# mdw771/beyond_dof

Hardware: AMD Instinct MI355X
Metric: multislice fwd+adjoint slice-steps/s (full Adam iteration: rotation, forward, loss, adjoint, gradient exchange, regulariser+Adam) (higher is better)
Workload: dtype f32

## Files before the change

### beyond_dof_amd/_lib.py

```python
import ctypes
import os
import sys

import numpy as np

_HERE = os.path.dirname(os.path.abspath(__file__))
LIB_PATH = os.environ.get('BDOF_LIB') or os.path.join(_HERE, 'libbdof.so')

DET_NONE, DET_NEAR, DET_FAR = 0, 1, 2
VARIANT_NUMPY_SKIP_LAST, VARIANT_TF_ALL = 0, 1
LOSS_LSQ, LOSS_POISSON = 0, 1
CFG_GRAD, CFG_GENERIC, CFG_NO_RESIDENT, CFG_ALWAYS_RESIDENT, CFG_RECOMPUTE, CFG_NO_GROT, CFG_ADJOINT64 = 1, 2, 4, 8, 16, 32, 64
K_ROW_FWD, K_COL_PROP, K_ROW_BWD, K_LOSS, K_ROT_ADJ, K_ADAM = range(6)
KERNEL_CLASS_NAMES = ['row_fwd', 'col_prop', 'row_bwd', 'loss', 'rot_adjoint', 'adam']

_c_int_p = ctypes.POINTER(ctypes.c_int)
_c_float_p = ctypes.POINTER(ctypes.c_float)
_vp = ctypes.c_void_p

_SIGNATURES = {
    'bdof_ctx_create': (ctypes.c_int, [ctypes.POINTER(_vp), ctypes.c_int, _vp]),
    'bdof_ctx_destroy': (None, [_vp]),
    'bdof_last_error': (ctypes.c_char_p, [_vp]),
    'bdof_sync': (ctypes.c_int, [_vp]),
# ... 61 lines not shown
    'bdof_grot': (_vp, [_vp]),
    'bdof_tape_slot': (_vp, [_vp, ctypes.c_int]),
    'bdof_modulation_table': (ctypes.c_int, [_vp, ctypes.POINTER(_vp), ctypes.POINTER(ctypes.c_size_t), ctypes.POINTER(ctypes.c_double)]),
    'bdof_rotation_adjoint': (ctypes.c_int, [_vp, ctypes.c_int, _vp, _vp, ctypes.c_int, ctypes.c_float]),
    'bdof_rotation_adjoint_rows': (ctypes.c_int, [_vp, ctypes.c_int, _vp, _vp, ctypes.c_int, ctypes.c_int, ctypes.c_int, ctypes.c_float]),
    'bdof_rotate_bilinear': (ctypes.c_int, [_vp, _vp, ctypes.c_int, ctypes.c_int, ctypes.c_int, _vp, ctypes.c_int, _vp]),
    'bdof_set_object_bilinear': (ctypes.c_int, [_vp, _vp, ctypes.c_int, ctypes.c_int, ctypes.c_int, _vp, ctypes.c_int, ctypes.c_int]),
    'bdof_rotate_bilinear_adjoint': (ctypes.c_int, [_vp, _vp, ctypes.c_int, ctypes.c_int, ctypes.c_int, _vp, ctypes.c_int, _vp, ctypes.c_int, ctypes.c_int, ctypes.c_int, ctypes.c_float]),
    'bdof_window_rotation_adjoint': (ctypes.c_int, [_vp, ctypes.c_int, ctypes.c_int, _vp, _vp, _vp, ctypes.c_int, ctypes.c_float]),
    'bdof_adam_step': (ctypes.c_int, [_vp, _vp, _vp, _vp, _vp, _vp, _vp, ctypes.c_int, ctypes.c_int, ctypes.c_int]
                       + [ctypes.c_float] * 8 + [ctypes.c_int, ctypes.c_int]),
    'bdof_adam_step_slab': (ctypes.c_int, [_vp, _vp, _vp, _vp, _vp, _vp, _vp, ctypes.c_int, ctypes.c_int, ctypes.c_int]
                            + [ctypes.c_float] * 8 + [ctypes.c_int] * 4),
    'bdof_rotation_adjoint_adam': (ctypes.c_int, [_vp, ctypes.c_int, _vp, _vp, ctypes.c_int, ctypes.c_int, ctypes.c_int, ctypes.c_float,
                                                  _vp, _vp, _vp, _vp, _vp, ctypes.c_int, ctypes.c_int, ctypes.c_int]
                                   + [ctypes.c_float] * 8 + [ctypes.c_int, ctypes.c_int]),
    'bdof_regularizer_value': (ctypes.c_int, [_vp, _vp, ctypes.c_int, ctypes.c_int, ctypes.c_int, ctypes.POINTER(ctypes.c_double)]),
    'bdof_mask_shrink': (ctypes.c_int, [_vp, _vp, _vp, ctypes.c_size_t, ctypes.c_float]),
    'bdof_gather_fields': (ctypes.c_int, [_vp, _vp, _vp, _vp, ctypes.c_int, ctypes.c_size_t]),
    'bdof_set_streams': (ctypes.c_int, [_vp, ctypes.c_int]),
    'bdof_batch_groups': (ctypes.c_int, [_vp, ctypes.c_int]),
    'bdof_set_sweep_fusion': (ctypes.c_int, [_vp, ctypes.c_int]),
    'bdof_sweep_fused': (ctypes.c_int, [_vp]),
    'bdof_profile_enable': (ctypes.c_int, [_vp, ctypes.c_int]),
    'bdof_profile_read': (ctypes.c_int, [_vp, ctypes.c_int, _c_int_p, ctypes.POINTER(ctypes.c_double)]),
    'bdof_malloc': (ctypes.c_int, [ctypes.POINTER(_vp), ctypes.c_size_t]),
    'bdof_device_mem': (ctypes.c_int, [_vp, ctypes.POINTER(ctypes.c_size_t), ctypes.POINTER(ctypes.c_size_t)]),
    'bdof_ctx_malloc': (ctypes.c_int, [_vp, ctypes.POINTER(_vp), ctypes.c_size_t]),
    'bdof_comm_unique_id': (ctypes.c_int, [_vp, ctypes.c_size_t]),
    'bdof_comm_create': (ctypes.c_int, [ctypes.POINTER(_vp), ctypes.c_int, ctypes.c_int, ctypes.c_int, _vp, ctypes.c_size_t]),
    'bdof_comm_destroy': (None, [_vp]),
    'bdof_comm_last_error': (ctypes.c_char_p, [_vp]),
    'bdof_comm_size': (ctypes.c_int, [_vp]),
    'bdof_comm_rank': (ctypes.c_int, [_vp]),
    'bdof_allreduce_grad': (ctypes.c_int, [_vp, _vp, _vp, ctypes.c_size_t, _c_int_p]),
    'bdof_reduce_scatter_grad': (ctypes.c_int, [_vp, _vp, _vp, ctypes.c_size_t, _c_int_p]),
    'bdof_allgather_volume': (ctypes.c_int, [_vp, _vp, _vp, ctypes.c_size_t, _c_int_p]),
    'bdof_bcast_volume': (ctypes.c_int, [_vp, _vp, _vp, ctypes.c_size_t, ctypes.c_int, _c_int_p]),
    'bdof_comm_wait': (ctypes.c_int, [_vp, _vp, ctypes.c_int]),
    'bdof_comm_sync': (ctypes.c_int, [_vp]),
    'bdof_free': (ctypes.c_int, [_vp]),
    'bdof_memcpy_h2d': (ctypes.c_int, [_vp, _vp, _vp, ctypes.c_size_t]),
    'bdof_memcpy_d2h': (ctypes.c_int, [_vp, _vp, _vp, ctypes.c_size_t]),
    'bdof_memset': (ctypes.c_int, [_vp, _vp, ctypes.c_int, ctypes.c_size_t]),
    'bdof_memcpy_d2d': (ctypes.c_int, [_vp, _vp, _vp, ctypes.c_size_t]),
}
# ... 153 lines not shown
```

### beyond_dof_amd/csrc/bdof_capi.hip

```cpp
#include <hip/hip_runtime.h>
#include <hip/hip_ext.h>
#include <cmath>
#include <algorithm>
#include <complex>
#include <cstdio>
#include <cstdlib>
#include <cstring>
#include <string>
#include <vector>

#include "../../include/bdof.h"
#include "bdof_steps.h"
#include "bdof_kernels.h"
#include "bdof_conv2.h"
#include "bdof_generic.h"
#include "bdof_field.h"
#include "bdof_conv64.h"
#include "bdof_resident.h"
#include "bdof_comm.h"
#include <rocfft/rocfft.h>
#include <map>
#include <array>

#define BDOF_ERR_ARG (-1)
// ... 70 lines not shown
    DevBuf<double2> cdet64;
    bool resident = false;
    DevBuf<cf> hsT, hdetT, twR, res_carrier;
    DevBuf<cf> pstack, pdet, pdetT;
    DevBuf<double2> pdet64, pdetT64;
    std::map<std::array<int, 4>, PlanPair> plans;
    FftExec fft;
    bool have_h64 = false;
    DevBuf<double2> g64, hs64, hdet64;
};

struct bdof_ctx : Workspace {
    int device = 0;
    hipStream_t stream = nullptr;
    bool own_stream = false;
    hipStream_t side[BDOF_MAX_GROUPS - 1] = {};
    int n_side = -1;
    std::vector<hipStream_t> side_all;
    hipEvent_t ev_fork = nullptr, ev_join[BDOF_MAX_GROUPS - 1] = {};
    hipEvent_t timer[BDOF_N_TIMERS] = {};
    int n_streams = -1;
    int fusion = 0;
    int fused_last = 0;
    int ncu = 256;
    int NY = 0, NX = 0, S = 0, Bmax = 0;
    bool with_grad = false;
    bool recompute = false;
    int tw_dither = 0;
    const float2* obj_src = nullptr;
    const int *adj_off = nullptr, *adj_order = nullptr;
    const cf* range_car = nullptr;
    int range_car_B = 0, range_car_z0 = 0;
    DevBuf<double2> car_scratch;
    hipStream_t aux = nullptr;
    hipEvent_t ev_aux_fork = nullptr, ev_aux_join = nullptr;
    FftExec fft_aux;
    bool aux_pending = false;
    bool c64_tf = false;
    std::complex<double> c64_ksum{1.0, 0.0};
    double c64_k = 0.0;
    int gpsi_B = 0;
    int npartial = 0;
    float k = 0.f;
    float k_fft = 0.f;
    std::complex<double> h00{1.0, 0.0}, hdet00{1.0, 0.0}, a0{0.0, 0.0};
    std::complex<double> cbm1{0.0, 0.0};
// ... 345 lines not shown
    sq_of(c, (unsigned)z, a.sq);
    DISPATCH_N(c->NY, with_bool(a.pz != nullptr, [&](auto PF) {
        BDOF_LAUNCH(ps, (k_row_fwd<N_, false, true, PF, true>), dim3(rows_grid<N_>(c, g.B, c->NX)), dim3(BDOF_THREADS), 0, g.st, a);
    }));
}

static void launch_row_prop(bdof_ctx* c, const Group& g, const cf* in, cf* out, const cf* h, float scale, int conj_h, int key, int cls = BDOF_K_COL_PROP) {
    ProfScope ps(c, cls, g.st, true);
    const unsigned tick = (unsigned)key;
    if (h == c->hs && c->hs_copies > 0) h = c->hs_d + (size_t)(tick % (unsigned)c->hs_copies) * c->NX * c->NY;
    RowPropArgs a{sub_field(c, g, in), sub_field(c, g, out), h, g.B, c->NY, scale, conj_h, tw_of(c, c->twX, c->NX, tick)};
    sq_of(c, tick, a.sq);
    DISPATCH_N(c->NX, {
        BDOF_LAUNCH(ps, (k_row_prop<N_, false>), dim3(rows_grid<N_>(c, g.B, c->NY)), dim3(BDOF_THREADS), 0, g.st, a);
    });
}

static int fused_mode(const bdof_ctx* c) {
    if (c->fusion < 1 || c->sep_copies < 1 || c->recompute || c->bin != 1 || c->pstack || c->range_car) return 0;
    if (c->det_mode == BDOF_DET_FAR || c->obj.xoff || c->obj.yoff || c->gpsi0) return 0;
    if (c->S < 4 || (c->S & 1) || c->NX > 512 || c->NY > 512) return 0;
    return 1;
}
static void launch_slice(bdof_ctx* c, const Group& g, int z, const cf* in, cf* out, cf* phi) {
    ProfScope ps(c, BDOF_K_ROW_FWD, g.st, true);
    const bool xl = (z & 1) != 0;
    const int N = xl ? c->NX : c->NY, R = xl ? c->NY : c->NX;
    const cf* tw = xl ? c->twX : c->twY;
    const cf* h = xl ? c->hx_d : c->hy_d;
    const unsigned lead = (unsigned)(z > 0 ? z - 1 : 0), trail = (unsigned)z, D = (unsigned)c->sep_copies;
    SliceArgs a{sub_field(c, g, in), c->probe, sub_field(c, g, out), sub_field(c, g, phi), sub_obj(c, g), g.B, R, z, carrier_at(c, z), cshift_at(c, z),
                tw_of(c, tw, N, lead), tw_of(c, tw, N, trail), h + (size_t)(lead % D) * N, h + (size_t)(trail % D) * N};
    sq_of(c, lead, a.sq_lead);
    sq_of(c, trail, a.sq_trail);
    if (xl) {
        DISPATCH_N_512(N, BDOF_LAUNCH(ps, (k_slice_x<N_>), dim3(rows_grid<N_>(c, g.B, R)), dim3(BDOF_THREADS), 0, g.st, a));
    } else {
        DISPATCH_N_512(N, with_bool(z == 0, [&](auto FIRST) { with_bool(z == c->S - 2, [&](auto TAIL) {
            BDOF_LAUNCH(ps, (k_slice_y<N_, FIRST, TAIL>), dim3(rows_grid<N_>(c, g.B, R)), dim3(BDOF_THREADS), 0, g.st, a);
        }); }));
    }
}

struct GradTarget {
    float2* grot = nullptr;
    int S_ = 0, z_ = 0;
    cf* gpsi = nullptr;
};
static void launch_row_bwd(bdof_ctx* c, const Group& g, int z, const cf* gin, const cf* tape, cf* gout, int hist = 0, float tape_scale = 1.f,
                           const GradTarget* gt = nullptr) {
    ProfScope ps(c, BDOF_K_ROW_BWD, g.st, true);
    float2* grot = gt && gt->grot ? gt->grot + (size_t)g.b0 * gt->S_ * c->NX * c->NY : c->grot + (size_t)g.b0 * c->S * c->NX * c->NY;
    RowBwdArgs a{sub_field(c, g, gin), hist == 2 ? c->probe : sub_field(c, g, tape), sub_field(c, g, gout),
                 grot, sub_obj(c, g), g.B, c->NX, z, c->k, carrier_at(c, z), tw_of(c, c->twY, c->NY, (unsigned)z),
                 slice_carrier_field(c, z), adj_carrier_at(c, g, steps(c).steps_back(z)), cshift_at(c, z), carrier_phi_at(c, z), tape_scale,
                 gt && gt->gpsi ? sub_field(c, g, gt->gpsi) : (z == 0 ? sub_field<cf>(c, g, c->gpsi0) : nullptr),
                 gt && gt->grot ? gt->S_ : c->S, gt && gt->grot ? gt->z_ : steps(c).first_slice(z)};
    sq_of(c, (unsigned)z, a.sq);
    const int form = a.ac.gcar ? 2 : a.pz ? 1 : 0;
    if (c->bin > 1) {
        DISPATCH_N(c->NY, with_bool(hist == 2, [&](auto H2) { with_int<3>(form, [&](auto FORM) {
            BDOF_LAUNCH(ps, (k_row_bwd<N_, H2 ? 2 : 1, FORM == 1, FORM == 2, true>), dim3(rows_grid<N_>(c, g.B, c->NX)), dim3(BDOF_THREADS), 0, g.st, a);
// ... 40 lines not shown
    a.twiddle = c->twX;
    int grid = 0;
    DISPATCH_N(c->NX, grid = rows_grid<N_>(c, g.B, c->NY); with_bool(meas && loss_is_poisson(c), [&](auto PSN) {
        hipLaunchKernelGGL((k_row_loss<N_, true, true, PSN>), dim3(grid), dim3(BDOF_THREADS), 0, g.st, a);
    }));
    return grid;
}

struct DetRoute {
    bool far;
    const cf* in;
    float in_scale;
    const cf* h;
    const cf* pfield;
};
static DetRoute det_route(const bdof_ctx* c) {
    const bool tf_all = c->variant == BDOF_VARIANT_TF_ALL;
    if (c->det_mode == BDOF_DET_FAR) return DetRoute{true, c->bufA, 1.f, nullptr, c->pdetT};
    if (c->det_mode == BDOF_DET_NONE && !tf_all) return DetRoute{false, c->bufA, 1.f / (float)c->NY, nullptr, c->pdet};
    return DetRoute{false, c->bufB, 1.f, c->det_mode == BDOF_DET_NONE ? c->hs : tf_all ? c->hcomb : c->hdet, c->pdet};
}

enum { TAPE_NONE = 0, TAPE_HISTORY = 1, TAPE_LAST = 2 };
static void forward_sweep(bdof_ctx* c, const Split& split, int tape_mode, bool fused = false) {
    const size_t fld = (size_t)c->Bmax * c->NX * c->NY;
    const DetRoute dr = det_route(c);
    const int nz = n_steps(c);
    for (int z = 0; z < nz; ++z) {
        const cf* in = nullptr;
        if (z > 0) in = tape_mode == TAPE_HISTORY ? c->tape + (size_t)steps(c).tape_read(z) * fld : c->bufB;
        const bool last = z == nz - 1;
        if (fused && last) in = c->tape + (size_t)z * fld;
        if (fused && !last) {
            for (const Group& g : split) {
                launch_slice(c, g, z, (z & 1) ? c->bufA : c->bufB, (z & 1) ? c->bufB : c->bufA, c->tape + (size_t)z * fld);
                if (z == nz - 2) launch_row_prop(c, g, c->bufA, c->tape + (size_t)(nz - 1) * fld, c->hx_rows, 1.f, 0, z, BDOF_K_LOSS);
            }
            continue;
        }
        cf* phi = tape_mode == TAPE_LAST && last ? c->tape : nullptr;
        for (const Group& g : split) {
            if (!last) {
                launch_row_fwd(c, g, z, in, c->bufA, true, phi);
                launch_row_prop(c, g, c->bufA, tape_mode == TAPE_HISTORY ? c->tape + (size_t)steps(c).tape_write(z) * fld : c->bufB, c->hs, 1.f, 0, z);
            } else {
                launch_row_fwd(c, g, z, in, c->bufA, dr.far || dr.h, phi);
                if (dr.h) launch_row_prop(c, g, c->bufA, c->bufB, dr.h, 1.f, 0, z, fused ? BDOF_K_LOSS : BDOF_K_COL_PROP);
            }
        }
    }
}

static void march_back(bdof_ctx* c, const Group& g, int z, int hist, const cf* phi, bool phi_real, bool step, bool march, cf* rc1, cf* rc2,
                       const GradTarget* gt = nullptr) {
    launch_row_bwd(c, g, z, c->bufB, phi, step ? c->bufA : nullptr, hist, 1.f, gt);
    if (step) launch_row_prop(c, g, c->bufA, c->bufB, c->hs, 1.f, 1, z - 1);
    if (march) {
        launch_row_unmod(c, g, z, phi, rc2, phi_real, 1.f);
        launch_row_prop(c, g, rc2, rc1, c->hs, 1.f, 1, z - 1);
    }
}

static void adjoint_sweep(bdof_ctx* c, const Split& split, bool fused) {
    const size_t fld = (size_t)c->Bmax * c->NX * c->NY;
    const int nz = n_steps(c);
    for (int z = nz - 1; z >= 0; --z) {
        const bool top = z == nz - 1;
        for (const Group& g : split) {
            if (c->recompute) {
                march_back(c, g, z, z == 0 ? 2 : top ? 0 : 3, top ? c->tape : c->tape + fld, top, z > 0, z > 1, c->tape + fld, c->tape + 2 * fld);
                continue;
            }
            if (fused) launch_row_bwd(c, g, z, c->bufB, c->tape + (size_t)z * fld, z > 0 ? c->bufA : nullptr, top ? 1 : 0);
            else launch_row_bwd(c, g, z, c->bufB, z > 0 ? c->tape + (size_t)steps(c).tape_read(z) * fld : nullptr, z > 0 ? c->bufA : nullptr, z > 0 ? 1 : 2);
            if (z > 0) launch_row_prop(c, g, c->bufA, c->bufB, c->hs, 1.f, 1, z - 1);
        }
    }
}

static int modulation_room(bdof_ctx* c, size_t n, bool mean) {
    HIPC(c, c->mod.room(n));
    if (mean) HIPC(c, c->cbar_dev.room((size_t)c->ncu * 16 + 1));
    return 0;
}
static int modulation_bound(bdof_ctx* c, size_t at, bool mean) {
    std::complex<double> cb(0.0, 0.0);
    if (mean) {
        double2 m;
        HIPC(c, hipMemcpyAsync(&m, c->cbar_dev + at, sizeof(double2), hipMemcpyDeviceToHost, c->stream));
        HIPC(c, hipStreamSynchronize(c->stream));
        cb = std::complex<double>(m.x, m.y);
        if (c->bin > 1) cb = std::pow(1.0 + cb, c->bin) - 1.0;
    }
// ... 1386 lines not shown
    if (i < nz - 1) {
        launch_loss_real(c, whole(c, B), wave_plane(c, carrier_z(c, i + 1), slice_carrier_field(c, i + 1)), c->tape + (size_t)i * fld, nullptr, false,
                         (cf*)out, nullptr, 1.f, 1.f);
    } else {
        if (!c->last_valid)
            return fail(c, BDOF_ERR_STATE, "the last slice's wave is only kept after bdof_forward(keep_tape=1) with the numpy_skip_last variant");
        launch_loss_real(c, whole(c, B), wave_plane(c, carrier_z(c, nz - 1) * (1.0 + c->cbm1), slice_carrier_field(c, nz - 1)), c->bufA, nullptr, false,
                         (cf*)out, nullptr, 1.f / c->NY, 1.f);
    }
    return launched(c);
}

int bdof_loss_grad(bdof_ctx* c, int B, const int* angle_of_b, const int* xoff, const int* yoff, const float* meas, void* out_wave) {
    int r = check_ready(c, B);
    if (r) return r;
    if (!meas) return BDOF_ERR_ARG;
    if (c->meas_dev && (c->det_mode == BDOF_DET_FAR || c->pstack))
        return fail(c, BDOF_ERR_STATE, "bdof_set_meas_mode(1) needs a real-space detector and a scalar carrier");
    if (!c->with_grad || !c->grot) return fail(c, BDOF_ERR_STATE, "bdof_loss_grad needs bdof_configure(with_grad=1) with the gradient workspace (not flag 32)");
    if ((r = need_angles(c, angle_of_b))) return r;
    if ((r = begin_batch(c, angle_of_b, xoff, yoff, c->k_fft))) return r;
    c->gpsi_src = c->gpsi0;
    c->gpsi_B = B;
    c->fused_last = 0;
    if (use_resident(c, B)) {
        if ((r = resident_run(c, B, meas, out_wave, true))) return r;
        c->tape_valid = c->last_valid = false;
        return 0;
    }
    if (c->generic) {
        if ((r = generic_loss_grad(c, B, meas, out_wave))) return r;
        c->tape_valid = c->last_valid = false;
        c->gpsi_src = c->bufA;
        return launched(c);
    }
    Split split;
    if ((r = split.open(c, B, c->NX, 16))) return r;
    const bool fused = fused_mode(c) != 0;
    c->fused_last = fused ? 1 : 0;
    forward_sweep(c, split, c->recompute ? TAPE_LAST : TAPE_HISTORY, fused);
    c->tape_valid = false;
    c->last_valid = false;
    int npart = 0;
    const DetRoute dr = det_route(c);
    for (const Group& g : split) {
        const DetPlane det = det_plane(c, g, B, dr.pfield);
        if (dr.far) {
            npart += launch_loss_far(c, g, det, dr.in, c->bufB, (cf*)out_wave, meas, 1.f, 1.f, npart);
        } else if (!dr.h) {
            npart += launch_loss_real(c, g, det, dr.in, c->bufB, false, (cf*)out_wave, meas, dr.in_scale, dr.in_scale, npart);
        } else {
            npart += launch_loss_real(c, g, det, dr.in, c->bufA, true, (cf*)out_wave, meas, 1.f, 1.f, npart);
            launch_row_prop(c, g, c->bufA, c->bufB, dr.h, 1.f, 1, n_steps(c) - 1, fused ? BDOF_K_LOSS : BDOF_K_COL_PROP);
        }
    }
    adjoint_sweep(c, split, fused);
    if ((r = split.close(c))) return r;
    hipLaunchKernelGGL(k_sum_partials, dim3(1), dim3(256), 0, c->stream, c->partial, npart,
                       1.0 / ((double)B * c->NX * c->NY), c->loss_dev);
    return launched(c);
}


int bdof_set_conv(bdof_ctx* c, const float* ky, const float* kx, int ks, double e_re, double e_im, double ksum_re,
                  double ksum_im, double k) {
    if (int rb = need_unbinned(c, "bdof_set_conv")) return rb;
    if (!c || !ky || !kx) return BDOF_ERR_ARG;
    if (int r = need_configured(c)) return r;
    if (ks < 1 || ks > BDOF_CONV_MAXK || ks % 2 == 0) return fail(c, BDOF_ERR_ARG, "kernel_size must be odd and <= 33");
    if (c->generic || c->NX % BDOF_CONV_TX || c->NY % BDOF_CONV_TY)
        return fail(c, BDOF_ERR_SIZE, "the conv propagator needs power-of-two wavefields (tiles are 32 x 64)");
    HIPC(c, hipSetDevice(c->device));
    c->c64_tf = false; c->c64_ks = 0;
    for (int i = 0; i < ks; ++i) {
        c->taps.ky[i] = make_float2(ky[2 * i], ky[2 * i + 1]);
        c->taps.kx[i] = make_float2(kx[2 * i], kx[2 * i + 1]);
    }
    c->taps.e = make_float2((float)e_re, (float)e_im);
    c->taps.ks = ks;
// ... 609 lines not shown
    if (!c || !dst || !src || !idx || B < 1) return BDOF_ERR_ARG;
    if (bytes_per_field % 4) return fail(c, BDOF_ERR_SIZE, "bdof_gather_fields: fields must be multiples of 4 bytes");
    HIPC(c, hipSetDevice(c->device));
    if (bytes_per_field % 16) {
        const size_t n4 = bytes_per_field / 4;
        const int gx4 = (int)std::min<size_t>((n4 + 255) / 256, 64);
        hipLaunchKernelGGL(k_gather_fields4, dim3(gx4, B < 1024 ? B : 1024), dim3(256), 0, c->stream, (float*)dst, (const float*)src, idx, B, n4);
        return launched(c);
    }
    const size_t n16 = bytes_per_field / 16;
    const int gx = (int)std::min<size_t>((n16 + 255) / 256, 64);
    hipLaunchKernelGGL(k_gather_fields, dim3(gx, B < 1024 ? B : 1024), dim3(256), 0, c->stream, (float4*)dst, (const float4*)src, idx, B, n16);
    return launched(c);
}

int bdof_set_sweep_fusion(bdof_ctx* c, int mode) {
    if (!c) return BDOF_ERR_ARG;
    if (mode < 0 || mode > 2) return fail(c, BDOF_ERR_ARG, "bdof_set_sweep_fusion: mode must be 0, 1 or 2");
    c->fusion = std::min(mode, 1);
    return 0;
}
int bdof_sweep_fused(bdof_ctx* c) { return c ? c->fused_last : 0; }

int bdof_set_streams(bdof_ctx* c, int n) {
    if (!c) return -1;
    if (n == 0 || n > BDOF_MAX_GROUPS) return fail(c, -2, "bdof_set_streams: n must be -1 or 1..4");
    c->n_streams = n < 0 ? -1 : n;
    return 0;
}

int bdof_batch_groups(bdof_ctx* c, int B) {
    if (!c || B < 1 || !c->NX) return -1;
    if (c->generic) return 1;
    Group g[BDOF_MAX_GROUPS];
    return batch_groups(c, B, c->NX, 16, g);
}

int bdof_profile_enable(bdof_ctx* c, int enable) {
    if (!c) return BDOF_ERR_ARG;
    HIPC(c, hipStreamSynchronize(c->stream));
    prof_collect(c);
    if (enable) { for (int i = 0; i < BDOF_K_COUNT; ++i) { c->prof_ms[i] = 0; c->prof_n[i] = 0; c->prof_seen[i] = 0; } }
    c->prof = enable != 0;
    c->prof_stride = enable > 1 ? enable : 1;
    return 0;
}
// ... 200 lines not shown
```

### beyond_dof_amd/csrc/bdof_kernels.h

```cpp
#pragma once
#include "bdof_fft.h"

#define BDOF_THREADS 512

template <int N> struct RowCfg {
    static constexpr int T = N / 8;
    static constexpr int RPP = BDOF_THREADS / T;
    static constexpr int TILE = RPP > 16 ? RPP : 16;
    static constexpr int PASSES = TILE / RPP;
    static constexpr int NPAD = N + N / 16;
    static constexpr int RS = ((NPAD + 29) / 32) * 32 + 2;
    static constexpr int LDS_CF = TILE * RS;
    static constexpr int MIN_WAVES = N >= 1024 ? 2 : 4;
};

template <int T> struct RowLds {
    cf* base;
    __device__ __forceinline__ int slot(int i) const { return i + (i >> 4); }
    __device__ __forceinline__ cf ld_at(int base_slot, int c) const { return base[base_slot + c + (c >> 4)]; }
    __device__ __forceinline__ void st_at(int base_slot, int c, cf v) { base[base_slot + c + (c >> 4)] = v; }
    __device__ __forceinline__ void sync_w2r() { sync(); }
    __device__ __forceinline__ void sync_r2w() { sync(); }
    __device__ __forceinline__ void sync() {
        if constexpr (T <= 64) {
// ... 747 lines not shown
            cf* pdst = a.phi_out + (size_t)(row0 + r) * NY;
#pragma unroll
            for (int m = 0; m < 8; ++m) pdst[tid + m * C::T] = u[m];
            tw_select(tw, smem_tw[1], smem_tail[1], sqt, tid);
            if constexpr (TAIL) {
                line_fft_partial<NY, -1, 1, false>(u, tw, tid, lds);
            } else {
#pragma unroll
                for (int m = 0; m < 8; ++m) hv[m] = a.h_trail[tid + m * C::T];
                line_fft<NY, -1, 1, false>(u, tw, tid, lds);
#pragma unroll
                for (int m = 0; m < 8; ++m) u[m] = cmul(u[m], hv[m]);
                line_fft_partial<NY, +1, 2, false>(u, tw, tid, lds);
            }
        }
        __syncthreads();
        cf* dst = a.out + (size_t)b * NY * NX + x0;
        if constexpr (TAIL) transposed_tail_mul<NY, -1, 1>(smem, dst, NX, a.h_trail, smem_tail[1], sqt);
        else transposed_tail<NY, +1, 2, false>(smem, dst, NX, 1.f, smem_tail[1], sqt);
        __syncthreads();
    }
}

template <int NX>
__global__ __launch_bounds__(BDOF_THREADS, RowCfg<NX>::MIN_WAVES) void k_slice_x(SliceArgs a) {
    typedef RowCfg<NX> C;
    typedef FftPlan<NX> P;
    __shared__ cf smem[C::LDS_CF];
    __shared__ cf smem_tw[2][FftTw<NX>::LDS_CNT];
    __shared__ cf smem_tail[2][7 * C::T];
    const int tid = threadIdx.x % C::T, rl = threadIdx.x / C::T;
    const float sql[2] = {a.sq_lead[0], a.sq_lead[1]}, sqt[2] = {a.sq_trail[0], a.sq_trail[1]};
    __shared__ int s_src[NX];
    FftTw<NX> tw;
    tw_fill<NX>(a.tw_lead, smem_tw[0], smem_tail[0]);
    tw_fill<NX>(a.tw_trail, smem_tw[1], smem_tail[1]);
    __syncthreads();
    const ObjView o = a.obj;
    const int NY = a.R;
    const int ntiles = a.B * NY / C::TILE;
    for (int tile = blockIdx.x; tile < ntiles; tile += gridDim.x) {
        const int row0 = tile * C::TILE;
        const int b = row0 / NY, y0 = row0 - b * NY;
        const ObjRows rows = obj_rows_of(o, b, a.z, NX);
        cf* const pdst = a.phi_out + (size_t)b * NX * NY;
        const int src_mine = (int)threadIdx.x < NX ? obj_rows_rel(rows, threadIdx.x) : -1;
#pragma nounroll
        for (int pass = 0; pass < C::PASSES; ++pass) {
            const int r = pass * C::RPP + rl;
            RowLds<C::T> lds{smem + r * C::RS};
            cf u[8], hv[8];
            const cf* src = a.in + (size_t)(row0 + r) * NX;
#pragma unroll
            for (int m = 0; m < 8; ++m) u[m] = src[tid + m * C::T];
#pragma unroll
            for (int m = 0; m < 8; ++m) hv[m] = a.h_lead[tid + m * C::T];
            tw_select(tw, smem_tw[0], smem_tail[0], sql, tid);
            line_fft<NX, -1, 1, false>(u, tw, tid, lds);
#pragma unroll
            for (int m = 0; m < 8; ++m) u[m] = cmul(u[m], hv[m]);
            line_fft_partial<NX, +1, 2, false>(u, tw, tid, lds);
        }
        if ((int)threadIdx.x < NX) s_src[threadIdx.x] = src_mine;
        __syncthreads();
        cf v[C::PASSES][8];
#pragma unroll
        for (int pass = 0; pass < C::PASSES; ++pass) {
            const int q = threadIdx.x + pass * BDOF_THREADS;
            const int r = q % C::TILE, j = q / C::TILE;
            RowLds<C::T> lds{smem + r * C::RS};
            const int yg = y0 + r, yc = min(max(yg, 0), o.volNY - 1);
            float2 db[8];
#pragma unroll
            for (int m = 0; m < 8; ++m) {
                const int srel = s_src[j + m * C::T];
                const float2 t = o.vol[(size_t)(rows.plain0 + max(srel, 0)) * o.volNY + yc];
                const bool in = srel >= 0 && yg == yc;
                db[m] = make_float2(in ? t.x : 0.f, in ? t.y : 0.f);
            }
            last_stage<NX, +1, 2, false>(v[pass], j, lds, smem_tail[0], sql);
#pragma unroll
            for (int m = 0; m < 8; ++m) {
                v[pass][m] = modulate_eps_s(v[pass][m], a.carrier, db[m], a.cshift);
                pdst[(unsigned)((j + m * C::T) * NY + yg)] = v[pass][m];
            }
            tw.sq = sqt;
            stage_compute<NX, -1, P::R0, 1, 0, 1, false>(v[pass], tw, j);
        }
        __syncthreads();
#pragma unroll
        for (int pass = 0; pass < C::PASSES; ++pass) {
            const int q = threadIdx.x + pass * BDOF_THREADS;
            const int r = q % C::TILE, j = q / C::TILE;
            RowLds<C::T> lds{smem + r * C::RS};
            stage_write<NX, P::R0, 1>(v[pass], j, lds);
        }
        __syncthreads();
#pragma nounroll
        for (int pass = 0; pass < C::PASSES; ++pass) {
            const int r = pass * C::RPP + rl;
            RowLds<C::T> lds{smem + r * C::RS};
            cf u[8], hv[8];
#pragma unroll
            for (int m = 0; m < 8; ++m) hv[m] = a.h_trail[tid + m * C::T];
            tw_select(tw, smem_tw[1], smem_tail[1], sqt, tid);
            line_fft_rest<NX, -1, 1, false>(u, tw, tid, lds);
#pragma unroll
            for (int m = 0; m < 8; ++m) u[m] = cmul(u[m], hv[m]);
            line_fft_partial<NX, +1, 2, false>(u, tw, tid, lds);
        }
        __syncthreads();
        transposed_tail<NX, +1, 2, false>(smem, a.out + (size_t)b * NX * NY + y0, NY, 1.f, smem_tail[1], sqt);
        __syncthreads();
    }
}

struct AdamArgs {
    const float2* x_old;
    float2* x_new;
    const float2* g;
    float2* m;
    float2* v;
    const float* mask;
    int NXv, NZv, NYv;
    float g_scale;
    float alpha_d, alpha_b, gamma;
    float lr, b1, b2, eps, inv_bc1, inv_bc2;
    float om_b1, om_b2;
    int clip;
    int x0, x1;
};
// ... 941 lines not shown
```

### beyond_dof_amd/engine.py

```python
import ctypes
import os

import numpy as np

from . import _lib
from ._lib import DeviceBuffer
from . import util

_VARIANT = {'numpy_skip_last': _lib.VARIANT_NUMPY_SKIP_LAST, 'tf_all': _lib.VARIANT_TF_ALL}
_LOSS = {'lsq': _lib.LOSS_LSQ, 'poisson': _lib.LOSS_POISSON}


def check_loss(loss_type, poisson_multiplier):
    if loss_type not in _LOSS:
        raise ValueError("loss_type must be 'lsq' or 'poisson'")
    if not float(poisson_multiplier) > 0:
        raise ValueError('poisson_multiplier must be > 0')


def check_poisson_path(loss_type, poisson_multiplier, propagator):
    check_loss(loss_type, poisson_multiplier)
    if loss_type == 'poisson' and propagator != 'fft':
        raise ValueError("loss_type='poisson' runs on the transfer-function propagator (propagator='fft') only")

# ... 387 lines not shown
        self.ctx.check(self.lib.bdof_rotation_adjoint(self.h, B, a.ptr, _lib._ptr(gvol_buf), int(accumulate), float(scale)))
        self.ctx.sync()

    def adam_step(self, x_old, x_new, g, m, v, mask, shape_xzy, i_batch, lr, g_scale=1.0, alpha_d=0.0, alpha_b=0.0,
                  gamma=0.0, b1=0.9, b2=0.999, eps=1e-8, clip=True, slab=None):
        nxv, nzv, nyv = [int(s) for s in shape_xzy]
        x0, nx = (0, nxv) if slab is None else (int(slab[0]), int(slab[1]))
        self.ctx.check(self.lib.bdof_adam_step_slab(self.h, _lib._ptr(x_old), _lib._ptr(x_new), _lib._ptr(g), _lib._ptr(m),
                                                    _lib._ptr(v), _lib._ptr(mask), nxv, nzv, nyv, g_scale, alpha_d, alpha_b,
                                                    gamma, lr, b1, b2, eps, int(i_batch), int(clip), x0, nx))

    def stream_ptr(self):
        return int(self.lib.bdof_stream(self.h) or 0)

    def set_streams(self, n=-1):
        self.ctx.check(self.lib.bdof_set_streams(self.h, int(n)))

    def batch_groups(self, B):
        return int(self.lib.bdof_batch_groups(self.h, int(B)))

    def set_sweep_fusion(self, mode):
        self.ctx.check(self.lib.bdof_set_sweep_fusion(self.h, int(mode)))

    @property
    def sweep_fused(self):
        return int(self.lib.bdof_sweep_fused(self.h))

    def profile_enable(self, on=True, stride=1):
        self.ctx.check(self.lib.bdof_profile_enable(self.h, int(stride) if on else 0))

    def profile_read(self):
        res = {}
        for cls, name in enumerate(_lib.KERNEL_CLASS_NAMES):
            n = ctypes.c_int(0)
            ms = ctypes.c_double(0)
            self.ctx.check(self.lib.bdof_profile_read(self.h, cls, ctypes.byref(n), ctypes.byref(ms)))
            res[name] = (n.value, ms.value)
        return res

    def sync(self):
        self.ctx.sync()
```

### beyond_dof_amd/solver.py

```python
import ctypes
import os

import numpy as np

from . import _lib
from ._lib import DeviceBuffer
from . import util
from .comm import PseudoComm
from .engine import MultisliceEngine, RESIDENT_SIZES, check_poisson_path, check_binning_path


class _VolumeSolver(object):

    lookahead = 2

    def _init_volume(self):
        shape = (self.dim_x, self.dim_z, self.dim_y, 2)
        self.x = [DeviceBuffer.zeros(self.ctx, shape, np.float32), DeviceBuffer.zeros(self.ctx, shape, np.float32)]
        self.cur = 0
        self.g = DeviceBuffer.zeros(self.ctx, shape, np.float32)
        self.m = DeviceBuffer.zeros(self.ctx, shape, np.float32)
        self.v = DeviceBuffer.zeros(self.ctx, shape, np.float32)
        self.mask = None
        self.nvox = self.dim_x * self.dim_z * self.dim_y
# ... 4 lines not shown
        self._g_shards = None
        self._g_stale = False
        self.probe = None
        self._pgrad = None
        self.meas = None
        self.meas_all = None
        self.comm.attach(self.ctx)

    def _upload_rotation_tables(self, coord_ls):
        if coord_ls is None:
            coord_ls = util.rotation_lookup([self.dim_y, self.dim_x, self.dim_z], self.n_theta)
        tables = util.device_rotation_tables(coord_ls, self.dim_x, self.dim_z)
        self.tab, self.off, self.order = [DeviceBuffer.from_host(self.ctx, t) for t in tables]

    def _bind_volume(self):
        self.eng.set_volume(self.x[self.cur], self.dim_x * self.dim_z, self.dim_y, self.tab, self.dim_x, self.n_theta)

    def set_sweep_fusion(self, mode):
        self.eng.set_sweep_fusion(mode)

    @property
    def sweep_fused(self):
        return self.eng.sweep_fused

    def set_volume(self, obj_delta, obj_beta):
        self.x[self.cur].upload(util.volume_to_rows(obj_delta, obj_beta))
        self._bind_volume()

    def get_volume(self):
        self.ctx.sync()
        return util.rows_to_volume(self.x[self.cur].download())

    def set_mask(self, mask):
        self.mask = None if mask is None else DeviceBuffer.from_host(
            self.ctx, np.ascontiguousarray(np.asarray(mask, dtype=np.float32).transpose(1, 2, 0)))

    def reset_moments(self):
        lib, h = self.ctx.lib, self.ctx.handle
        self.ctx.check(lib.bdof_memset(h, self.m.ptr, 0, self.m.nbytes))
        self.ctx.check(lib.bdof_memset(h, self.v.ptr, 0, self.v.nbytes))
        self._acc = 0
        self._epoch_plan = None

    def bcast_volume(self, root=0):
        if self.comm.size > 1:
            self.comm.bcast_device(self.ctx, self.x[self.cur], root)
# ... 234 lines not shown
                 coord_ls=None, propagator='fft', kernel_size=17, recompute=False, rotation='nearest', theta=None, adjoint64=None,
                 detector_kernel='TF', loss_type='lsq', poisson_multiplier=2e6, slice_binning=1):
        check_poisson_path(loss_type, poisson_multiplier, propagator)
        check_binning_path(slice_binning, propagator, 'float64' if adjoint64 else None, rotation if rotation == 'bilinear' else 'nearest')
        self.conv = propagator == 'conv'
        self.bilinear = rotation == 'bilinear'
        if adjoint64 not in (None, False, True, 'first'):
            raise ValueError("adjoint64 must be None, False, True or 'first'")
        if adjoint64 and rotation == 'bilinear' and (self.conv or adjoint64 == 'first'):
            raise ValueError("the float64 paths (adjoint64='first'; propagator='conv') run with the lookup-table rotation")
        self.f64 = 'first' if adjoint64 == 'first' else (True if (adjoint64 is True and self.conv) else None)
        adjoint64 = adjoint64 is True and not self.conv
        if rotation not in ('nearest', 'bilinear'):
            raise ValueError("rotation must be 'nearest' or 'bilinear'")
        if self.bilinear and theta is None:
            raise ValueError("rotation='bilinear' needs the projection angles theta")
        self.dim_y, self.dim_x, self.dim_z = int(dim_y), int(dim_x), int(dim_z)
        self.n_theta, self.mb = int(n_theta), int(minibatch_size)
        self.comm = comm or PseudoComm()
        self.eng = MultisliceEngine(self.dim_y, self.dim_x, self.dim_z, self.mb, with_grad=True, device=device, stream=stream,
                                    recompute=recompute, adjoint64=adjoint64, slice_binning=slice_binning)
        self.ctx = self.eng.ctx
        self.eng.set_sweep_fusion(1)
        self.eng.set_loss(loss_type, poisson_multiplier)
        self.eng.set_physics(energy_ev, psize_cm, free_prop_cm, variant=variant, detector_kernel=detector_kernel)
        if self.conv:
            self.eng.set_conv(energy_ev, psize_cm, kernel_size)
        if probe_real is None:
            probe_real, probe_imag = np.ones((dim_y, dim_x)), np.zeros((dim_y, dim_x))
        self.eng.set_probe(probe_real, probe_imag)
        if self.f64:
            self._enable_f64()
        if self.bilinear:
            th = np.asarray(theta, dtype=np.float64)
            assert len(th) == self.n_theta
            H, W = self.dim_x, self.dim_z
            c, sn = np.cos(th), np.sin(th)
            self.rot_prm = np.stack([c, sn, ((W - 1) - (c * (W - 1) - sn * (H - 1))) / 2.0, ((H - 1) - (sn * (W - 1) + c * (H - 1))) / 2.0], axis=1)
            self.prm_buf = DeviceBuffer(self.ctx, self.mb * 32, np.float64, (self.mb, 4))
            self.tab = self.off = self.order = None
        else:
            self._upload_rotation_tables(coord_ls)
        self._init_volume()
        self.meas_stage = DeviceBuffer(self.ctx, self.mb * self.dim_x * self.dim_y * 4, np.float32,
                                       (self.mb, self.dim_x, self.dim_y))
        self.angle_buf = DeviceBuffer(self.ctx, self.mb * 4, np.int32, (self.mb,))
# ... 220 lines not shown
```

### include/bdof.h

```cpp
#ifndef BDOF_H
#define BDOF_H
#include <stddef.h>
#ifdef __cplusplus
extern "C" {
#endif

typedef struct bdof_ctx bdof_ctx;

enum { BDOF_DET_NONE = 0, BDOF_DET_NEAR = 1, BDOF_DET_FAR = 2 };
enum { BDOF_VARIANT_NUMPY_SKIP_LAST = 0, BDOF_VARIANT_TF_ALL = 1 };
enum { BDOF_K_ROW_FWD = 0, BDOF_K_COL_PROP = 1, BDOF_K_ROW_BWD = 2, BDOF_K_LOSS = 3, BDOF_K_ROT_ADJ = 4, BDOF_K_ADAM = 5, BDOF_K_COUNT = 6 };
enum { BDOF_CFG_GRAD = 1, BDOF_CFG_GENERIC = 2, BDOF_CFG_NO_RESIDENT = 4, BDOF_CFG_ALWAYS_RESIDENT = 8, BDOF_CFG_RECOMPUTE = 16,
       BDOF_CFG_NO_GROT = 32, BDOF_CFG_ADJOINT64 = 64 };

int bdof_ctx_create(bdof_ctx** out, int device, void* stream);
void bdof_ctx_destroy(bdof_ctx* ctx);
const char* bdof_last_error(const bdof_ctx* ctx);
int bdof_sync(bdof_ctx* ctx);
void* bdof_stream(bdof_ctx* ctx);
int bdof_device_count(void);

int bdof_twiddle_tables(int N, int D, float* out);
int bdof_device_pci_bus_id(int device, char* out, int len);
int bdof_timer_mark(bdof_ctx* ctx, int slot);
// ... 105 lines not shown
int bdof_adam_step(bdof_ctx* ctx, const void* x_old, void* x_new, const void* g, void* m, void* v, const float* mask,
                   int NXv, int NZv, int NYv, float g_scale, float alpha_d, float alpha_b, float gamma,
                   float lr, float b1, float b2, float eps, int i_batch, int clip);
int bdof_adam_step_slab(bdof_ctx* ctx, const void* x_old, void* x_new, const void* g, void* m, void* v, const float* mask,
                        int NXv, int NZv, int NYv, float g_scale, float alpha_d, float alpha_b, float gamma,
                        float lr, float b1, float b2, float eps, int i_batch, int clip, int x0, int nx);

int bdof_rotation_adjoint_adam(bdof_ctx* ctx, int B, const int* angle_of_b, void* gvol, int row0, int n_rows, int accumulate, float scale,
                               const void* x_old, void* x_new, void* m, void* v, const float* mask, int NXv, int NZv, int NYv,
                               float g_scale, float alpha_d, float alpha_b, float gamma, float lr, float b1, float b2, float eps,
                               int i_batch, int clip);

int bdof_gather_fields(bdof_ctx* ctx, void* dst, const void* src, const int* idx, int B, size_t bytes_per_field);

int bdof_regularizer_value(bdof_ctx* ctx, const void* x, int NXv, int NZv, int NYv, double* sums);

int bdof_mask_shrink(bdof_ctx* ctx, const void* x, float* mask, size_t n, float thresh);

int bdof_set_streams(bdof_ctx* ctx, int n);
int bdof_batch_groups(bdof_ctx* ctx, int B);

int bdof_set_sweep_fusion(bdof_ctx* ctx, int mode);
int bdof_sweep_fused(bdof_ctx* ctx);

int bdof_profile_enable(bdof_ctx* ctx, int enable);
int bdof_profile_read(bdof_ctx* ctx, int kernel_class, int* n_launches, double* total_ms);

typedef struct bdof_comm bdof_comm;
int bdof_comm_unique_id(void* id, size_t bytes);
int bdof_comm_create(bdof_comm** out, int device, int nranks, int rank, const void* id, size_t bytes);
void bdof_comm_destroy(bdof_comm* comm);
const char* bdof_comm_last_error(const bdof_comm* comm);
int bdof_comm_size(const bdof_comm* comm);
int bdof_comm_rank(const bdof_comm* comm);
int bdof_allreduce_grad(bdof_comm* comm, bdof_ctx* ctx, void* buf, size_t count, int* ticket);
int bdof_reduce_scatter_grad(bdof_comm* comm, bdof_ctx* ctx, void* buf, size_t count_per_rank, int* ticket);
int bdof_allgather_volume(bdof_comm* comm, bdof_ctx* ctx, void* buf, size_t count_per_rank, int* ticket);
int bdof_bcast_volume(bdof_comm* comm, bdof_ctx* ctx, void* buf, size_t count, int root, int* ticket);
int bdof_comm_wait(bdof_comm* comm, bdof_ctx* ctx, int ticket);
int bdof_comm_sync(bdof_comm* comm);

int bdof_ctx_malloc(bdof_ctx* ctx, void** ptr, size_t bytes);
int bdof_device_mem(bdof_ctx* ctx, size_t* free_bytes, size_t* total_bytes);
int bdof_malloc(void** ptr, size_t bytes);
int bdof_free(void* ptr);
int bdof_memcpy_h2d(bdof_ctx* ctx, void* dst, const void* src, size_t bytes);
// ... 9 lines not shown
```

Before: 206,300.

## Fuse adjoint slice step into single per-slice kernel with blocked tape layout

Adds fused adjoint slice kernels (k_slice_y_adj / k_slice_x_adj) that do the backward propagation, the object-gradient write and the modulation adjoint for two half-steps in one launch, mirroring the existing fused forward slice kernel. When adjoint fusion is on, the forward x-slice kernel stores its tape in a row-blocked layout so the adjoint kernel can read it contiguously. The solver enables this by default. The aim is fewer launches and fewer global round trips per slice in the adjoint sweep, at the cost of heavier kernels and a second tape layout that has to stay consistent between forward and backward.

```diff
diff --git a/beyond_dof_amd/_lib.py b/beyond_dof_amd/_lib.py
--- a/beyond_dof_amd/_lib.py
+++ b/beyond_dof_amd/_lib.py
@@ -107,6 +107,8 @@
     'bdof_batch_groups': (ctypes.c_int, [_vp, ctypes.c_int]),
     'bdof_set_sweep_fusion': (ctypes.c_int, [_vp, ctypes.c_int]),
     'bdof_sweep_fused': (ctypes.c_int, [_vp]),
+    'bdof_set_adjoint_fusion': (ctypes.c_int, [_vp, ctypes.c_int]),
+    'bdof_adjoint_fused': (ctypes.c_int, [_vp]),
     'bdof_profile_enable': (ctypes.c_int, [_vp, ctypes.c_int]),
     'bdof_profile_read': (ctypes.c_int, [_vp, ctypes.c_int, _c_int_p, ctypes.POINTER(ctypes.c_double)]),
     'bdof_malloc': (ctypes.c_int, [ctypes.POINTER(_vp), ctypes.c_size_t]),
diff --git a/beyond_dof_amd/csrc/bdof_capi.hip b/beyond_dof_amd/csrc/bdof_capi.hip
--- a/beyond_dof_amd/csrc/bdof_capi.hip
+++ b/beyond_dof_amd/csrc/bdof_capi.hip
@@ -116,6 +116,8 @@
     int n_streams = -1;
     int fusion = 0;
     int fused_last = 0;
+    int adj_fusion = 0;
+    int adj_fused_last = 0;
     int ncu = 256;
     int NY = 0, NX = 0, S = 0, Bmax = 0;
     bool with_grad = false;
@@ -507,7 +509,7 @@
     if (c->S < 4 || (c->S & 1) || c->NX > 512 || c->NY > 512) return 0;
     return 1;
 }
-static void launch_slice(bdof_ctx* c, const Group& g, int z, const cf* in, cf* out, cf* phi) {
+static void launch_slice(bdof_ctx* c, const Group& g, int z, const cf* in, cf* out, cf* phi, bool blk = false) {
     ProfScope ps(c, BDOF_K_ROW_FWD, g.st, true);
     const bool xl = (z & 1) != 0;
     const int N = xl ? c->NX : c->NY, R = xl ? c->NY : c->NX;
@@ -519,10 +521,32 @@
     sq_of(c, lead, a.sq_lead);
     sq_of(c, trail, a.sq_trail);
     if (xl) {
-        DISPATCH_N_512(N, BDOF_LAUNCH(ps, (k_slice_x<N_>), dim3(rows_grid<N_>(c, g.B, R)), dim3(BDOF_THREADS), 0, g.st, a));
+        DISPATCH_N_512(N, with_bool(blk, [&](auto BLK) {
+            BDOF_LAUNCH(ps, (k_slice_x<N_, BLK>), dim3(rows_grid<N_>(c, g.B, R)), dim3(BDOF_THREADS), 0, g.st, a);
+        }));
     } else {
         DISPATCH_N_512(N, with_bool(z == 0, [&](auto FIRST) { with_bool(z == c->S - 2, [&](auto TAIL) {
             BDOF_LAUNCH(ps, (k_slice_y<N_, FIRST, TAIL>), dim3(rows_grid<N_>(c, g.B, R)), dim3(BDOF_THREADS), 0, g.st, a);
+        }); }));
+    }
+}
+
+static void launch_slice_adj(bdof_ctx* c, const Group& g, int z, const cf* in, cf* out, const cf* phi) {
+    ProfScope ps(c, BDOF_K_ROW_BWD, g.st, true);
+    const bool xl = (z & 1) != 0;
+    const int N = xl ? c->NX : c->NY, R = xl ? c->NY : c->NX;
+    const cf* tw = xl ? c->twX : c->twY;
+    const cf* h = xl ? c->hx_d : c->hy_d;
+    const unsigned lead = (unsigned)z, trail = (unsigned)(z > 0 ? z - 1 : 0), D = (unsigned)c->sep_copies;
+    SliceAdjArgs a{sub_field(c, g, in), sub_field(c, g, phi), sub_field(c, g, out), c->grot + (size_t)g.b0 * c->S * c->NX * c->NY, sub_obj(c, g), g.B, R, z,
+                   c->k, carrier_phi_at(c, z), tw_of(c, tw, N, lead), tw_of(c, tw, N, trail), h + (size_t)(lead % D) * N, h + (size_t)(trail % D) * N};
+    sq_of(c, lead, a.sq_lead);
+    sq_of(c, trail, a.sq_trail);
+    if (xl) {
+        DISPATCH_N_512(N, BDOF_LAUNCH(ps, (k_slice_x_adj<N_>), dim3(rows_grid<N_>(c, g.B, R)), dim3(BDOF_THREADS), 0, g.st, a));
+    } else {
+        DISPATCH_N_512(N, with_bool(z == c->S - 2, [&](auto HEAD) { with_bool(z == 0, [&](auto LAST) {
+            BDOF_LAUNCH(ps, (k_slice_y_adj<N_, HEAD, LAST>), dim3(rows_grid<N_>(c, g.B, R)), dim3(BDOF_THREADS), 0, g.st, a);
         }); }));
     }
 }
@@ -609,7 +633,7 @@
 }
 
 enum { TAPE_NONE = 0, TAPE_HISTORY = 1, TAPE_LAST = 2 };
-static void forward_sweep(bdof_ctx* c, const Split& split, int tape_mode, bool fused = false) {
+static void forward_sweep(bdof_ctx* c, const Split& split, int tape_mode, bool fused = false, bool adj_fused = false) {
     const size_t fld = (size_t)c->Bmax * c->NX * c->NY;
     const DetRoute dr = det_route(c);
     const int nz = n_steps(c);
@@ -620,7 +644,7 @@
         if (fused && last) in = c->tape + (size_t)z * fld;
         if (fused && !last) {
             for (const Group& g : split) {
-                launch_slice(c, g, z, (z & 1) ? c->bufA : c->bufB, (z & 1) ? c->bufB : c->bufA, c->tape + (size_t)z * fld);
+                launch_slice(c, g, z, (z & 1) ? c->bufA : c->bufB, (z & 1) ? c->bufB : c->bufA, c->tape + (size_t)z * fld, adj_fused);
                 if (z == nz - 2) launch_row_prop(c, g, c->bufA, c->tape + (size_t)(nz - 1) * fld, c->hx_rows, 1.f, 0, z, BDOF_K_LOSS);
             }
             continue;
@@ -648,7 +672,7 @@
     }
 }
 
-static void adjoint_sweep(bdof_ctx* c, const Split& split, bool fused) {
+static void adjoint_sweep(bdof_ctx* c, const Split& split, bool fused, bool adj_fused = false) {
     const size_t fld = (size_t)c->Bmax * c->NX * c->NY;
     const int nz = n_steps(c);
     for (int z = nz - 1; z >= 0; --z) {
@@ -656,6 +680,10 @@
         for (const Group& g : split) {
             if (c->recompute) {
                 march_back(c, g, z, z == 0 ? 2 : top ? 0 : 3, top ? c->tape : c->tape + fld, top, z > 0, z > 1, c->tape + fld, c->tape + 2 * fld);
+                continue;
+            }
+            if (adj_fused && !top) {
+                launch_slice_adj(c, g, z, (z & 1) ? c->bufA : c->bufB, (z & 1) ? c->bufB : c->bufA, c->tape + (size_t)z * fld);
                 continue;
             }
             if (fused) launch_row_bwd(c, g, z, c->bufB, c->tape + (size_t)z * fld, z > 0 ? c->bufA : nullptr, top ? 1 : 0);
@@ -2088,7 +2116,7 @@
     if ((r = begin_batch(c, angle_of_b, xoff, yoff, c->k_fft))) return r;
     c->gpsi_src = c->gpsi0;
     c->gpsi_B = B;
-    c->fused_last = 0;
+    c->fused_last = c->adj_fused_last = 0;
     if (use_resident(c, B)) {
         if ((r = resident_run(c, B, meas, out_wave, true))) return r;
         c->tape_valid = c->last_valid = false;
@@ -2103,8 +2131,10 @@
     Split split;
     if ((r = split.open(c, B, c->NX, 16))) return r;
     const bool fused = fused_mode(c) != 0;
+    const bool adj_fused = fused && c->adj_fusion != 0;
     c->fused_last = fused ? 1 : 0;
-    forward_sweep(c, split, c->recompute ? TAPE_LAST : TAPE_HISTORY, fused);
+    c->adj_fused_last = adj_fused ? 1 : 0;
+    forward_sweep(c, split, c->recompute ? TAPE_LAST : TAPE_HISTORY, fused, adj_fused);
     c->tape_valid = false;
     c->last_valid = false;
     int npart = 0;
@@ -2120,7 +2150,7 @@
             launch_row_prop(c, g, c->bufA, c->bufB, dr.h, 1.f, 1, n_steps(c) - 1, fused ? BDOF_K_LOSS : BDOF_K_COL_PROP);
         }
     }
-    adjoint_sweep(c, split, fused);
+    adjoint_sweep(c, split, fused, adj_fused);
     if ((r = split.close(c))) return r;
     hipLaunchKernelGGL(k_sum_partials, dim3(1), dim3(256), 0, c->stream, c->partial, npart,
                        1.0 / ((double)B * c->NX * c->NY), c->loss_dev);
@@ -2776,6 +2806,14 @@
 }
 int bdof_sweep_fused(bdof_ctx* c) { return c ? c->fused_last : 0; }
 
+int bdof_set_adjoint_fusion(bdof_ctx* c, int on) {
+    if (!c) return BDOF_ERR_ARG;
+    if (on < 0 || on > 1) return fail(c, BDOF_ERR_ARG, "bdof_set_adjoint_fusion: on must be 0 or 1");
+    c->adj_fusion = on;
+    return 0;
+}
+int bdof_adjoint_fused(bdof_ctx* c) { return c ? c->adj_fused_last : 0; }
+
 int bdof_set_streams(bdof_ctx* c, int n) {
     if (!c) return -1;
     if (n == 0 || n > BDOF_MAX_GROUPS) return fail(c, -2, "bdof_set_streams: n must be -1 or 1..4");
diff --git a/beyond_dof_amd/csrc/bdof_kernels.h b/beyond_dof_amd/csrc/bdof_kernels.h
--- a/beyond_dof_amd/csrc/bdof_kernels.h
+++ b/beyond_dof_amd/csrc/bdof_kernels.h
@@ -793,7 +793,7 @@
     }
 }
 
-template <int NX>
+template <int NX, bool BLK = false>
 __global__ __launch_bounds__(BDOF_THREADS, RowCfg<NX>::MIN_WAVES) void k_slice_x(SliceArgs a) {
     typedef RowCfg<NX> C;
     typedef FftPlan<NX> P;
@@ -814,7 +814,7 @@
         const int row0 = tile * C::TILE;
         const int b = row0 / NY, y0 = row0 - b * NY;
         const ObjRows rows = obj_rows_of(o, b, a.z, NX);
-        cf* const pdst = a.phi_out + (size_t)b * NX * NY;
+        cf* const pdst = a.phi_out + (BLK ? (size_t)row0 * NX : (size_t)b * NX * NY);
         const int src_mine = (int)threadIdx.x < NX ? obj_rows_rel(rows, threadIdx.x) : -1;
 #pragma nounroll
         for (int pass = 0; pass < C::PASSES; ++pass) {
@@ -853,7 +853,8 @@
 #pragma unroll
             for (int m = 0; m < 8; ++m) {
                 v[pass][m] = modulate_eps_s(v[pass][m], a.carrier, db[m], a.cshift);
-                pdst[(unsigned)((j + m * C::T) * NY + yg)] = v[pass][m];
+                if constexpr (BLK) pdst[(unsigned)(q + m * C::T * C::TILE)] = v[pass][m];
+                else pdst[(unsigned)((j + m * C::T) * NY + yg)] = v[pass][m];
             }
             tw.sq = sqt;
             stage_compute<NX, -1, P::R0, 1, 0, 1, false>(v[pass], tw, j);
@@ -878,6 +879,192 @@
             line_fft_rest<NX, -1, 1, false>(u, tw, tid, lds);
 #pragma unroll
             for (int m = 0; m < 8; ++m) u[m] = cmul(u[m], hv[m]);
+            line_fft_partial<NX, +1, 2, false>(u, tw, tid, lds);
+        }
+        __syncthreads();
+        transposed_tail<NX, +1, 2, false>(smem, a.out + (size_t)b * NX * NY + y0, NY, 1.f, smem_tail[1], sqt);
+        __syncthreads();
+    }
+}
+
+struct SliceAdjArgs {
+    const cf* in;
+    const cf* phi;
+    cf* out;
+    float2* grot;
+    ObjView obj;
+    int B, R, z;
+    float k;
+    cf carrier_phi;
+    const cf* tw_lead;
+    const cf* tw_trail;
+    const cf* h_lead;
+    const cf* h_trail;
+    float sq_lead[2], sq_trail[2];
+};
+
+template <int NY, bool HEAD, bool LAST>
+__global__ __launch_bounds__(BDOF_THREADS, RowCfg<NY>::MIN_WAVES) void k_slice_y_adj(SliceAdjArgs a) {
+    typedef RowCfg<NY> C;
+    __shared__ cf smem[C::LDS_CF];
+    __shared__ cf smem_tw[2][FftTw<NY>::LDS_CNT];
+    __shared__ cf smem_tail[2][7 * C::T];
+    const int tid = threadIdx.x % C::T, rl = threadIdx.x / C::T;
+    const float sql[2] = {a.sq_lead[0], a.sq_lead[1]}, sqt[2] = {a.sq_trail[0], a.sq_trail[1]};
+    FftTw<NY> tw;
+    tw_fill<NY>(a.tw_lead, smem_tw[0], smem_tail[0]);
+    if constexpr (!LAST) tw_fill<NY>(a.tw_trail, smem_tw[1], smem_tail[1]);
+    __syncthreads();
+    const int NX = a.R;
+    const int ntiles = a.B * NX / C::TILE;
+    for (int tile = blockIdx.x; tile < ntiles; tile += gridDim.x) {
+        const int row0 = tile * C::TILE;
+        const int b = row0 / NX, x0 = row0 - b * NX;
+#pragma nounroll
+        for (int pass = 0; pass < C::PASSES; ++pass) {
+            const int r = pass * C::RPP + rl;
+            const int x = x0 + r;
+            RowLds<C::T> lds{smem + r * C::RS};
+            const size_t off = (size_t)(row0 + r) * NY;
+            cf g[8], p[8], hv[8];
+            float2 db[8];
+#pragma unroll
+            for (int m = 0; m < 8; ++m) g[m] = a.in[off + tid + m * C::T];
+            if constexpr (!HEAD) {
+#pragma unroll
+                for (int m = 0; m < 8; ++m) hv[m] = a.h_lead[tid + m * C::T];
+            }
+            auto load_phi_and_table = [&]() {
+#pragma unroll
+                for (int m = 0; m < 8; ++m) p[m] = a.phi[off + tid + m * C::T];
+                load_obj_row(a.obj, obj_src_row(a.obj, b, x, a.z, NX), 0, tid, C::T, db);
+            };
+            tw_select(tw, smem_tw[0], smem_tail[0], sql, tid);
+            if constexpr (HEAD) {
+                load_phi_and_table();
+                line_fft<NY, +1, 1, false>(g, tw, tid, lds);
+            } else {
+                line_fft<NY, -1, 1, false>(g, tw, tid, lds);
+#pragma unroll
+                for (int m = 0; m < 8; ++m) g[m] = cmulc(g[m], hv[m]);
+                load_phi_and_table();
+                line_fft<NY, +1, 2, false>(g, tw, tid, lds);
+            }
+            float2* gdst = a.grot + (((size_t)b * a.obj.S + a.z) * NX + x) * NY;
+#pragma unroll
+            for (int m = 0; m < 8; ++m) {
+                const cf t = cmulc(g[m], cadd(p[m], a.carrier_phi));
+                gdst[tid + m * C::T] = make_float2(a.k * t.y, -a.k * t.x);
+                g[m] = cmulc(g[m], make_float2(1.f + db[m].x, db[m].y));
+            }
+            if constexpr (!LAST) {
+#pragma unroll
+                for (int m = 0; m < 8; ++m) hv[m] = a.h_trail[tid + m * C::T];
+                tw_select(tw, smem_tw[1], smem_tail[1], sqt, tid);
+                line_fft<NY, -1, 1, false>(g, tw, tid, lds);
+#pragma unroll
+                for (int m = 0; m < 8; ++m) g[m] = cmulc(g[m], hv[m]);
+                line_fft_partial<NY, +1, 2, false>(g, tw, tid, lds);
+            }
+        }
+        if constexpr (!LAST) {
+            __syncthreads();
+            transposed_tail<NY, +1, 2, false>(smem, a.out + (size_t)b * NY * NX + x0, NX, 1.f, smem_tail[1], sqt);
+            __syncthreads();
+        }
+    }
+}
+
+template <int NX>
+__global__ __launch_bounds__(BDOF_THREADS, RowCfg<NX>::MIN_WAVES) void k_slice_x_adj(SliceAdjArgs a) {
+    typedef RowCfg<NX> C;
+    typedef FftPlan<NX> P;
+    __shared__ cf smem[C::LDS_CF];
+    __shared__ cf smem_tw[2][FftTw<NX>::LDS_CNT];
+    __shared__ cf smem_tail[2][7 * C::T];
+    const int tid = threadIdx.x % C::T, rl = threadIdx.x / C::T;
+    const float sql[2] = {a.sq_lead[0], a.sq_lead[1]}, sqt[2] = {a.sq_trail[0], a.sq_trail[1]};
+    __shared__ int s_src[NX];
+    FftTw<NX> tw;
+    tw_fill<NX>(a.tw_lead, smem_tw[0], smem_tail[0]);
+    tw_fill<NX>(a.tw_trail, smem_tw[1], smem_tail[1]);
+    __syncthreads();
+    const ObjView o = a.obj;
+    const int NY = a.R;
+    const int ntiles = a.B * NY / C::TILE;
+    for (int tile = blockIdx.x; tile < ntiles; tile += gridDim.x) {
+        const int row0 = tile * C::TILE;
+        const int b = row0 / NY, y0 = row0 - b * NY;
+        const ObjRows rows = obj_rows_of(o, b, a.z, NX);
+        const cf* const psrc = a.phi + (size_t)row0 * NX;
+        float2* const gdst = a.grot + ((size_t)b * o.S + a.z) * NX * NY;
+        const int src_mine = (int)threadIdx.x < NX ? obj_rows_rel(rows, threadIdx.x) : -1;
+#pragma nounroll
+        for (int pass = 0; pass < C::PASSES; ++pass) {
+            const int r = pass * C::RPP + rl;
+            RowLds<C::T> lds{smem + r * C::RS};
+            cf u[8], hv[8];
+            const cf* src = a.in + (size_t)(row0 + r) * NX;
+#pragma unroll
+            for (int m = 0; m < 8; ++m) u[m] = src[tid + m * C::T];
+#pragma unroll
+            for (int m = 0; m < 8; ++m) hv[m] = a.h_lead[tid + m * C::T];
+            tw_select(tw, smem_tw[0], smem_tail[0], sql, tid);
+            line_fft<NX, -1, 1, false>(u, tw, tid, lds);
+#pragma unroll
+            for (int m = 0; m < 8; ++m) u[m] = cmulc(u[m], hv[m]);
+            line_fft_partial<NX, +1, 2, false>(u, tw, tid, lds);
+        }
+        if ((int)threadIdx.x < NX) s_src[threadIdx.x] = src_mine;
+        __syncthreads();
+        cf v[C::PASSES][8];
+#pragma unroll
+        for (int pass = 0; pass < C::PASSES; ++pass) {
+            const int q = threadIdx.x + pass * BDOF_THREADS;
+            const int r = q % C::TILE, j = q / C::TILE;
+            RowLds<C::T> lds{smem + r * C::RS};
+            const int yg = y0 + r, yc = min(max(yg, 0), o.volNY - 1);
+            float2 db[8];
+            cf p[8];
+#pragma unroll
+            for (int m = 0; m < 8; ++m) {
+                const int srel = s_src[j + m * C::T];
+                const float2 t = o.vol[(size_t)(rows.plain0 + max(srel, 0)) * o.volNY + yc];
+                const bool in = srel >= 0 && yg == yc;
+                db[m] = make_float2(in ? t.x : 0.f, in ? t.y : 0.f);
+            }
+#pragma unroll
+            for (int m = 0; m < 8; ++m) p[m] = psrc[(unsigned)(q + m * C::T * C::TILE)];
+            last_stage<NX, +1, 2, false>(v[pass], j, lds, smem_tail[0], sql);
+#pragma unroll
+            for (int m = 0; m < 8; ++m) {
+                const cf t = cmulc(v[pass][m], cadd(p[m], a.carrier_phi));
+                gdst[(unsigned)((j + m * C::T) * NY + yg)] = make_float2(a.k * t.y, -a.k * t.x);
+                v[pass][m] = cmulc(v[pass][m], make_float2(1.f + db[m].x, db[m].y));
+            }
+            tw.sq = sqt;
+            stage_compute<NX, -1, P::R0, 1, 0, 1, false>(v[pass], tw, j);
+        }
+        __syncthreads();
+#pragma unroll
+        for (int pass = 0; pass < C::PASSES; ++pass) {
+            const int q = threadIdx.x + pass * BDOF_THREADS;
+            const int r = q % C::TILE, j = q / C::TILE;
+            RowLds<C::T> lds{smem + r * C::RS};
+            stage_write<NX, P::R0, 1>(v[pass], j, lds);
+        }
+        __syncthreads();
+#pragma nounroll
+        for (int pass = 0; pass < C::PASSES; ++pass) {
+            const int r = pass * C::RPP + rl;
+            RowLds<C::T> lds{smem + r * C::RS};
+            cf u[8], hv[8];
+#pragma unroll
+            for (int m = 0; m < 8; ++m) hv[m] = a.h_trail[tid + m * C::T];
+            tw_select(tw, smem_tw[1], smem_tail[1], sqt, tid);
+            line_fft_rest<NX, -1, 1, false>(u, tw, tid, lds);
+#pragma unroll
+            for (int m = 0; m < 8; ++m) u[m] = cmulc(u[m], hv[m]);
             line_fft_partial<NX, +1, 2, false>(u, tw, tid, lds);
         }
         __syncthreads();
diff --git a/beyond_dof_amd/engine.py b/beyond_dof_amd/engine.py
--- a/beyond_dof_amd/engine.py
+++ b/beyond_dof_amd/engine.py
@@ -433,6 +433,13 @@
     def set_sweep_fusion(self, mode):
         self.ctx.check(self.lib.bdof_set_sweep_fusion(self.h, int(mode)))
 
+    def set_adjoint_fusion(self, on=True):
+        self.ctx.check(self.lib.bdof_set_adjoint_fusion(self.h, 1 if on else 0))
+
+    @property
+    def adjoint_fused(self):
+        return int(self.lib.bdof_adjoint_fused(self.h))
+
     @property
     def sweep_fused(self):
         return int(self.lib.bdof_sweep_fused(self.h))
diff --git a/beyond_dof_amd/solver.py b/beyond_dof_amd/solver.py
--- a/beyond_dof_amd/solver.py
+++ b/beyond_dof_amd/solver.py
@@ -50,6 +50,13 @@
     @property
     def sweep_fused(self):
         return self.eng.sweep_fused
+
+    def set_adjoint_fusion(self, on=True):
+        self.eng.set_adjoint_fusion(on)
+
+    @property
+    def adjoint_fused(self):
+        return self.eng.adjoint_fused
 
     def set_volume(self, obj_delta, obj_beta):
         self.x[self.cur].upload(util.volume_to_rows(obj_delta, obj_beta))
@@ -330,6 +337,7 @@
                                     recompute=recompute, adjoint64=adjoint64, slice_binning=slice_binning)
         self.ctx = self.eng.ctx
         self.eng.set_sweep_fusion(1)
+        self.eng.set_adjoint_fusion(True)
         self.eng.set_loss(loss_type, poisson_multiplier)
         self.eng.set_physics(energy_ev, psize_cm, free_prop_cm, variant=variant, detector_kernel=detector_kernel)
         if self.conv:
diff --git a/include/bdof.h b/include/bdof.h
--- a/include/bdof.h
+++ b/include/bdof.h
@@ -151,6 +151,8 @@
 
 int bdof_set_sweep_fusion(bdof_ctx* ctx, int mode);
 int bdof_sweep_fused(bdof_ctx* ctx);
+int bdof_set_adjoint_fusion(bdof_ctx* ctx, int on);
+int bdof_adjoint_fused(bdof_ctx* ctx);
 
 int bdof_profile_enable(bdof_ctx* ctx, int enable);
 int bdof_profile_read(bdof_ctx* ctx, int kernel_class, int* n_launches, double* total_ms);
```

New measurement: 237,000, median of 6. +14.9%, better.
